# Okrio/tinyrecurrentunet

Hardware: AMD Instinct MI355X
Metric: 16 kHz frames/sec (train step) (higher is better)
Workload: dtype f32; 1 GPU; config/tiny.json TRU-Net (C_in=4 incl. PCEN), 64 x 4 s 16 kHz pairs per GPU, n_fft 512 hop 128, full fp32 train step; mfma=fp32 forward, bf16x3 backward, fp32_mfma=bf16x3-bwd, frames_per_gpu=32064, global_batch=64, parallelism=dp1

## Files before the change

tinyrecurrentunet_amd/csrc/convt_bwd.hip:

```cpp
#include <type_traits>
#include "dma_common.hpp"
#include "x3_common.hpp"

namespace {

constexpr int CT_F = 32;
constexpr int CT_C = 64;
constexpr int CT_SET = CT_C * CT_F;
constexpr int CT_GRID = TRUNET_NUM_CU;
constexpr int CT_LO = CT_C * 16;

template <int K, int S>
constexpr bool ct_dzp() { return K == 3 && S == 1; }

__device__ __forceinline__ int ct_lo_off(int r, int pc) { return r * 16 + 2 * (pc ^ ((r >> 1) & 7)); }

__device__ __forceinline__ void ct_bstore(__amdgpu_buffer_rsrc_t r, int voff, int soff, float v) {
    __builtin_amdgcn_raw_buffer_store_b32(__builtin_bit_cast(int, v), r, voff, soff, 0);
}

template <int K, int S, bool X3>
struct CtLds {
    static constexpr bool DZP = X3 && ct_dzp<K, S>();
    static constexpr int RDZ = K + 2 * S;
    static constexpr int ZS = 2 * S;
    static constexpr int RS = 4;
    static constexpr int DZ = 0;
    static constexpr int ZST = DZ + RDZ * CT_SET;
    static constexpr int SRC = ZST + ZS * CT_SET;
    static constexpr int PART = SRC + RS * CT_SET;
    static constexpr int LO = PART + 2 * 2 * 16 * 64;
    static constexpr int COEF = LO + (DZP ? RDZ * CT_LO : 0);
    static constexpr size_t BYTES = COEF * sizeof(float) + 2 * CT_C * sizeof(f32x4);
    static_assert(BYTES <= 160 * 1024, "LDS");
};

template <int K>
struct CtWtF32 { float af[K][16]; };
template <int K>
struct CtWtX3 { u32x4 A0[K][2], A1[K][2], A2[K][2]; };

template <int K, int S, bool X3>
__global__ __launch_bounds__(512, X3 ? 1 : 2) void convt_bwd_kernel(const trunet_convt_bwd_args a) {
    using L = CtLds<K, S, X3>;
    constexpr int PAD = S / 2, RDZ = L::RDZ, ZS = L::ZS, RS = L::RS;
    constexpr bool DZP = L::DZP;
    extern __shared__ __attribute__((aligned(16))) float smem[];
    float* DZ = smem + L::DZ;
    float* ZST = smem + L::ZST;
    float* SRC = smem + L::SRC;
    float* PART = smem + L::PART;
    float* LO = smem + L::LO;
    f32x4* CA = (f32x4*)(smem + L::COEF);
    f32x4* CB = CA + CT_C;

    const int tid = threadIdx.x;
    const int lane = tid & 63;
    const int wave = __builtin_amdgcn_readfirstlane(tid >> 6);
    const int h = lane >> 5, c = lane & 31;
    const int NP = a.NP, Lin = a.Lin, Lout = a.Lout;

    for (int r = tid; r < CT_C; r += 512) {
        CA[r] = f32x4{a.ca[r], a.cb[r], a.cc[r], 0.f};
        CB[r] = f32x4{a.s_scale[r], a.s_shift[r], a.s_mean[r], 0.f};
    }
    const int nfc = NP / CT_F;
    const int c_begin = (int)(((long long)blockIdx.x * nfc) / gridDim.x);
    const int c_end = (int)(((long long)(blockIdx.x + 1) * nfc) / gridDim.x);
    __syncthreads();

    if (wave < 4) {
        const int cit = wave & 1, cot = wave >> 1;
        f32x16 acc[K];
#pragma unroll
        for (int k = 0; k < K; ++k)
#pragma unroll
            for (int r = 0; r < 16; ++r) acc[k][r] = 0.f;
        float bsum[2] = {0.f, 0.f};
        const int pc = lane & 7;
        int row_[2], lc_[2];
#pragma unroll
        for (int i = 0; i < 2; ++i) {
            row_[i] = 8 * (wave + 4 * i) + (lane >> 3);
            lc_[i] = pc ^ ((row_[i] >> 1) & 7);
        }
        const float sc_a = a.s_scale[cit * 32 + c], sh_a = a.s_shift[cit * 32 + c];

        auto issue = [&](int pa, int pb, int sq, int n0) __attribute__((always_inline)) -> int {
            int n = 0;
            for (int p = max(pa, 0); p < min(pb, Lout); ++p) {
                float* dst = DZ + (p % RDZ) * CT_SET;
                float* zst = ZST + (p % ZS) * CT_SET;
#pragma unroll
                for (int i = 0; i < 2; ++i) {
                    const size_t off = ((size_t)row_[i] * Lout + p) * NP + n0 + 4 * lc_[i];
                    __builtin_amdgcn_global_load_lds(a.dy + off, (lds_ptr_t)(dst + (wave + 4 * i) * 256), 16, 0, TRUNET_DMA_AUX);
                    __builtin_amdgcn_global_load_lds(a.z + off, (lds_ptr_t)(zst + (wave + 4 * i) * 256), 16, 0, TRUNET_DMA_AUX);
                }
                n += 4;
            }
            if (sq >= 0 && sq < Lin) {
                float* sdst = SRC + (sq % RS) * CT_SET;
#pragma unroll
                for (int i = 0; i < 2; ++i) {
                    const size_t off = ((size_t)row_[i] * Lin + sq) * NP + n0 + 4 * lc_[i];
                    __builtin_amdgcn_global_load_lds(a.src + off, (lds_ptr_t)(sdst + (wave + 4 * i) * 256), 16, 0, TRUNET_DMA_AUX);
                }
                n += 2;
            }
            return n;
        };
        auto prologue = [&](int pa, int pb, int n0) __attribute__((always_inline)) {
            for (int p = max(pa, 0); p < min(pb, Lout); ++p) {
                float* dst = DZ + (p % RDZ) * CT_SET;
                const float* zst = ZST + (p % ZS) * CT_SET;
#pragma unroll
                for (int i = 0; i < 2; ++i) {
                    const int o = row_[i] * CT_F + 4 * pc;
                    f32x4 v = *(f32x4*)(dst + o);
                    const f32x4 zz = *(const f32x4*)(zst + o);
                    const f32x4 k = CA[row_[i]];
                    float s = 0.f;
#pragma unroll
                    for (int e = 0; e < 4; ++e) {
                        v[e] = fmaf(k[0], v[e], fmaf(k[1], zz[e], k[2]));
                        if (n0 + 4 * lc_[i] + e >= a.N) v[e] = 0.f;
                        s += v[e];
                    }
                    bsum[i] += s;
                    if constexpr (DZP) {
                        unsigned h0, m0, l0, h1, m1, l1;
                        ctx_split2(v[0], v[1], h0, m0, l0);
                        ctx_split2(v[2], v[3], h1, m1, l1);
                        *(u32x4*)(dst + o) = u32x4{h0, h1, m0, m1};
                        *(u32x2*)(LO + (p % RDZ) * CT_LO + row_[i] * 16 + 2 * pc) = u32x2{l0, l1};
                    } else {
                        *(f32x4*)(dst + o) = v;
                    }
                }
            }
        };
        auto new_lo = [&](int q) { return q * S - PAD + K - S; };

        constexpr int NQQ = X3 ? CT_F / 16 : CT_F / 8, QQ_PRO = X3 ? 0 : 1;

        for (int ch = c_begin; ch < c_end; ++ch) {
            const int n0 = ch * CT_F;
            {
                const int pa = -PAD, pb = new_lo(1) + S;
                for (int p = pa; p < pb; p += ZS) {
                    issue(p, min(p + ZS, pb), p == pa ? 0 : (p == pa + ZS ? 1 : -1), n0);
                    asm volatile("s_waitcnt vmcnt(0)" ::: "memory");
                    prologue(p, min(p + ZS, pb), n0);
                    asm volatile("s_waitcnt lgkmcnt(0)" ::: "memory");
                }
                if (pb - pa <= ZS) { issue(0, 0, 1, n0); asm volatile("s_waitcnt vmcnt(0)" ::: "memory"); }
            }
            int n_last = issue(new_lo(2), new_lo(2) + S, 2, n0);
            asm volatile("s_waitcnt lgkmcnt(0)" ::: "memory");
            __builtin_amdgcn_s_barrier();
            asm volatile("" ::: "memory");
            for (int q = 0; q < Lin; ++q) {
                const float* Ssrc = SRC + (q % RS) * CT_SET;
                const int ra = cit * 32 + c, rb = cot * 32 + c;
#pragma unroll
                for (int qq = 0; qq < NQQ; ++qq) {
                    if constexpr (X3) {
                        f32x4 av0 = *(const f32x4*)(Ssrc + swz_off(ra, 4 * qq + 2 * h));
                        f32x4 av1 = *(const f32x4*)(Ssrc + swz_off(ra, 4 * qq + 2 * h + 1));
#pragma unroll
                        for (int e = 0; e < 4; ++e) {
                            av0[e] = fmaxf(fmaf(av0[e], sc_a, sh_a), 0.f);
                            av1[e] = fmaxf(fmaf(av1[e], sc_a, sh_a), 0.f);
                        }
                        u32x4 a0, a1, a2;
                        ctx_split8(av0, av1, a0, a1, a2);
#pragma unroll
                        for (int k = 0; k < K; ++k) {
                            const int p = q * S - PAD + k;
                            if (p >= 0 && p < Lout) {
                                const float* Dp = DZ + (p % RDZ) * CT_SET;
                                u32x4 b0, b1, b2;
                                if constexpr (DZP) {
                                    const float* Lp = LO + (p % RDZ) * CT_LO;
                                    const u32x4 q0 = *(const u32x4*)(Dp + swz_off(rb, 4 * qq + 2 * h));
                                    const u32x4 q1 = *(const u32x4*)(Dp + swz_off(rb, 4 * qq + 2 * h + 1));
                                    const u32x2 l0 = *(const u32x2*)(Lp + ct_lo_off(rb, 4 * qq + 2 * h));
                                    const u32x2 l1 = *(const u32x2*)(Lp + ct_lo_off(rb, 4 * qq + 2 * h + 1));
                                    b0 = u32x4{q0[0], q0[1], q1[0], q1[1]};
                                    b1 = u32x4{q0[2], q0[3], q1[2], q1[3]};
                                    b2 = u32x4{l0[0], l0[1], l1[0], l1[1]};
                                } else {
                                    const f32x4 bv0 = *(const f32x4*)(Dp + swz_off(rb, 4 * qq + 2 * h));
                                    const f32x4 bv1 = *(const f32x4*)(Dp + swz_off(rb, 4 * qq + 2 * h + 1));
                                    ctx_split8(bv0, bv1, b0, b1, b2);
                                }
                                CTX_MF6(acc[k], a0, a1, a2, b0, b1, b2);
                            }
                        }
                    } else {
                        f32x4 av = *(const f32x4*)(Ssrc + swz_off(ra, 2 * qq + h));
#pragma unroll
                        for (int e = 0; e < 4; ++e) av[e] = fmaxf(fmaf(av[e], sc_a, sh_a), 0.f);
#pragma unroll
                        for (int k = 0; k < K; ++k) {
                            const int p = q * S - PAD + k;
                            if (p >= 0 && p < Lout) {
                                const f32x4 bv = *(const f32x4*)(DZ + (p % RDZ) * CT_SET + swz_off(rb, 2 * qq + h));
#pragma unroll
                                for (int j = 0; j < 4; ++j)
                                    acc[k] = __builtin_amdgcn_mfma_f32_32x32x2f32(av[j], bv[j], acc[k], 0, 0, 0);
                            }
                        }
                    }
                    if (qq == QQ_PRO && q >= 1) {
                        wait_vmcnt_exact<31>(n_last);
                        prologue(new_lo(q + 1), new_lo(q + 1) + S, n0);
                    }
                }
                asm volatile("s_waitcnt lgkmcnt(0)" ::: "memory");
                __builtin_amdgcn_s_barrier();
                asm volatile("" ::: "memory");
                n_last = (q + 3 < Lin) ? issue(new_lo(q + 3), new_lo(q + 3) + S, q + 3, n0) : 0;
            }
            asm volatile("s_waitcnt vmcnt(0)" ::: "memory");
            __builtin_amdgcn_s_barrier();
            asm volatile("" ::: "memory");
        }
        float* img = a.w_partials + (size_t)blockIdx.x * a.w_numel;
#pragma unroll
        for (int k = 0; k < K; ++k)
#pragma unroll
            for (int r = 0; r < 16; ++r) {
                const int ci = cit * 32 + (r & 3) + 8 * (r >> 2) + 4 * h;
                const int co = cot * 32 + c;
                img[((size_t)ci * CT_C + co) * K + k] = acc[k][r];
            }
        if (a.b_partials) {
#pragma unroll
            for (int i = 0; i < 2; ++i) {
                float v = bsum[i];
                v += __shfl_xor(v, 4);
                v += __shfl_xor(v, 2);
                v += __shfl_xor(v, 1);
                if ((lane & 7) == 0) a.b_partials[(size_t)blockIdx.x * a.b_stride + a.b_off + row_[i]] = v;
            }
        }
    } else {
        const int jj = wave - 4;
        const int cit = jj & 1, chf = jj >> 1;
        const int trr = 8 * (lane >> 5) + ((lane & 15) >> 2), trp = 4 * ((lane >> 4) & 1) + (lane & 3);
        std::conditional_t<X3, CtWtX3<K>, CtWtF32<K>> wt;
        if constexpr (X3) {
            const float* wp = a.W + ((size_t)(cit * 32 + c) * CT_C + chf * 32 + 8 * h) * K;
#pragma unroll
            for (int k = 0; k < K; ++k)
#pragma unroll
                for (int ks = 0; ks < 2; ++ks) {
                    f32x4 w0, w1;
#pragma unroll
                    for (int j = 0; j < 4; ++j) {
                        w0[j] = wp[(size_t)(16 * ks + j) * K + k];
                        w1[j] = wp[(size_t)(16 * ks + 4 + j) * K + k];
                    }
                    ctx_split8(w0, w1, wt.A0[k][ks], wt.A1[k][ks], wt.A2[k][ks]);
                }
        } else {
            const float* wp = a.W + ((size_t)(cit * 32 + c) * CT_C + chf * 32 + h) * K;
#pragma unroll
            for (int kk = 0; kk < 16; ++kk)
#pragma unroll
                for (int k = 0; k < K; ++k) wt.af[k][kk] = wp[(size_t)(2 * kk) * K + k];
        }
        float st1[16], st2[16];
#pragma unroll
        for (int r = 0; r < 16; ++r) { st1[r] = 0.f; st2[r] = 0.f; }
        const size_t dstride = (size_t)Lin * NP;
        const int rowb = (int)(dstride * sizeof(float));
        const int voff = (int)((4 * h * dstride + c) * sizeof(float));

        f32x16 dacc;
        auto epilogue = [&](int q, int n0) __attribute__((always_inline)) {
            const float* P = PART + ((q & 1) * 2 + cit) * 16 * 64 + lane;
            const float* Ssrc = SRC + (q % RS) * CT_SET;
            const __amdgpu_buffer_rsrc_t ro = buffer_rsrc(a.dsrc + (size_t)(32 * cit) * dstride + (size_t)q * NP);
            const bool fin = n0 + c < a.N;
            const int nb = n0 * (int)sizeof(float);
#pragma unroll
            for (int r = 0; r < 16; ++r) {
                const int ml = (r & 3) + 8 * (r >> 2);
                const int row = cit * 32 + ml + 4 * h;
                const float zs = Ssrc[row * CT_F + 4 * ((c >> 2) ^ ((row >> 1) & 7)) + (c & 3)];
                const f32x4 k = CB[row];
                float val = dacc[r] + P[r * 64];
                val = (fmaf(k[0], zs, k[1]) > 0.f) ? val : 0.f;
                ct_bstore(ro, voff, ml * rowb + nb, val);
                const float x = fin ? val : 0.f;
                st1[r] += x;
                st2[r] = fmaf(x, zs - k[2], st2[r]);
            }
        };

        for (int ch = c_begin; ch < c_end; ++ch) {
            const int n0 = wave_uniform(ch * CT_F);
            asm volatile("" ::: "memory");
            __builtin_amdgcn_s_barrier();
            asm volatile("" ::: "memory");
            for (int q = 0; q < Lin; ++q) {
#pragma unroll
                for (int r = 0; r < 16; ++r) dacc[r] = 0.f;
#pragma unroll
                for (int k = 0; k < K; ++k) {
                    const int p = q * S - PAD + k;
                    if (p < 0 || p >= Lout) continue;
                    if constexpr (DZP) {
                        const float* Dq = DZ + (p % RDZ) * CT_SET;
                        const float* Lq = LO + (p % RDZ) * CT_LO;
#pragma unroll
                        for (int ks = 0; ks < 2; ++ks) {
                            const int r0 = chf * 32 + 16 * ks + trr;
                            const u32x2 h0 = lds_tr16(Dq + swz_off(r0, trp)), h1 = lds_tr16(Dq + swz_off(r0 + 4, trp));
                            const u32x2 m0 = lds_tr16(Dq + swz_off(r0, trp) + 2), m1 = lds_tr16(Dq + swz_off(r0 + 4, trp) + 2);
                            const u32x2 l0 = lds_tr16(Lq + ct_lo_off(r0, trp)), l1 = lds_tr16(Lq + ct_lo_off(r0 + 4, trp));
                            const u32x4 b0 = {h0[0], h0[1], h1[0], h1[1]}, b1 = {m0[0], m0[1], m1[0], m1[1]},
                                        b2 = {l0[0], l0[1], l1[0], l1[1]};
                            CTX_MF6(dacc, wt.A0[k][ks], wt.A1[k][ks], wt.A2[k][ks], b0, b1, b2);
                        }
                    } else if constexpr (X3) {
                        const float* Sb = DZ + (p % RDZ) * CT_SET + (chf * 32 + 8 * h) * CT_F + (c & 3);
                        const int cpc = c >> 2;
#pragma unroll
                        for (int ks = 0; ks < 2; ++ks) {
                            f32x4 x0, x1;
#pragma unroll
                            for (int j = 0; j < 4; ++j) {
                                x0[j] = Sb[(16 * ks + j) * CT_F + 4 * (cpc ^ ((4 * h + (j >> 1)) & 7))];
                                x1[j] = Sb[(16 * ks + 4 + j) * CT_F + 4 * (cpc ^ ((4 * h + 2 + (j >> 1)) & 7))];
                            }
                            u32x4 b0, b1, b2;
                            ctx_split8(x0, x1, b0, b1, b2);
                            CTX_MF6(dacc, wt.A0[k][ks], wt.A1[k][ks], wt.A2[k][ks], b0, b1, b2);
                        }
                    } else {
                        const float* Sb = DZ + (p % RDZ) * CT_SET + (chf * 32 + h) * CT_F + (c & 3);
                        const int cpc = c >> 2;
#pragma unroll
                        for (int kk = 0; kk < 16; ++kk) {
                            const float b = Sb[kk * (2 * CT_F) + 4 * (cpc ^ (kk & 7))];
                            dacc = __builtin_amdgcn_mfma_f32_32x32x2f32(wt.af[k][kk], b, dacc, 0, 0, 0);
                        }
                    }
                }
                if (chf == 1) {
                    float* P = PART + ((q & 1) * 2 + cit) * 16 * 64 + lane;
#pragma unroll
                    for (int r = 0; r < 16; ++r) P[r * 64] = dacc[r];
                }
                asm volatile("s_waitcnt lgkmcnt(0)" ::: "memory");
                __builtin_amdgcn_s_barrier();
                asm volatile("" ::: "memory");
                if (chf == 0) epilogue(q, n0);
            }
            asm volatile("s_waitcnt lgkmcnt(0)" ::: "memory");
            __builtin_amdgcn_s_barrier();
            asm volatile("" ::: "memory");
        }
        if (chf == 0 && a.partials) {
#pragma unroll
            for (int r = 0; r < 16; ++r) {
                const float s1 = half_wave_sum(st1[r]);
                const float s2 = half_wave_sum(st2[r]);
                const int row = cit * 32 + (r & 3) + 8 * (r >> 2) + 4 * h;
                if (c == 0) {
                    float* pp = a.partials + ((size_t)blockIdx.x * CT_C + row) * 2;
                    pp[0] = s1;
                    pp[1] = s2;
                }
            }
        }
    }
}

template <int K, int S, bool X3>
int ct_launch(const trunet_convt_bwd_args* h, hipStream_t st) {
    constexpr size_t lds = CtLds<K, S, X3>::BYTES;
    auto kern = convt_bwd_kernel<K, S, X3>;
    if (hipFuncSetAttribute((const void*)kern, hipFuncAttributeMaxDynamicSharedMemorySize, (int)lds) != hipSuccess)
        return TRUNET_ELAUNCH;
    hipLaunchKernelGGL(kern, dim3(CT_GRID), dim3(512), lds, st, *h);
    return trunet_launch_status();
}
template <int K, int S>
int ct_launch(const trunet_convt_bwd_args* h, hipStream_t st, bool x3) {
    return x3 ? ct_launch<K, S, true>(h, st) : ct_launch<K, S, false>(h, st);
}

}

extern "C" int trunet_convt_bwd_nparts(void) { return CT_GRID; }

extern "C" int trunet_convt_bwd(const trunet_convt_bwd_args* h, void* stream) {
    if (!h || !h->dy || !h->z || !h->ca || !h->cb || !h->cc || !h->src || !h->s_scale || !h->s_shift || !h->s_mean ||
        !h->W || !h->dsrc || !h->partials || !h->w_partials)
        return TRUNET_EINVAL;
    if (h->NP <= 0 || (h->NP % TRUNET_TILE_FRAMES) != 0 || h->N <= 0 || h->N > h->NP || h->Lin <= 0 || h->w_numel <= 0)
        return TRUNET_EINVAL;
    if (h->Ci != CT_C || h->Co != CT_C) return TRUNET_ENOTSUP;
    if (h->pad != h->S / 2 || h->Lout != (h->Lin - 1) * h->S - 2 * h->pad + h->K) return TRUNET_EINVAL;
    if ((size_t)h->Lin * h->NP * sizeof(float) * 36 >= ((size_t)1 << 31)) return TRUNET_ENOTSUP;
    hipStream_t st = (hipStream_t)stream;
    const bool x3 = (trunet_gemm_x3_enable(-1) & (TRUNET_X3_BWD | 8)) != 0;
    if (h->K == 3 && h->S == 1) return ct_launch<3, 1>(h, st, x3);
    if (h->K == 3 && h->S == 2) return ct_launch<3, 2>(h, st, x3);
    if (h->K == 5 && h->S == 2) return ct_launch<5, 2>(h, st, x3);
    return TRUNET_ENOTSUP;
}
```

Measured before the change: 760,900 frames/s.

## Extend pre-split dz layout to all bf16x3 convT bwd shapes, shorten stride-2 lookahead

Turns on the pre-split (hi/mid/lo) dz staging in LDS for every bf16x3 transposed-conv backward variant, not only K=3,S=1. The dW and dX loops no longer re-split dz fragments for each MFMA. For stride-2 X3 kernels the load lookahead drops from two steps to one, which shrinks the dz and source ring buffers to fit the extra LO buffer in LDS. The prologue is moved to the last qq iteration so the loads have more time to land. The shorter lookahead may expose more global-load latency.

```diff
diff --git a/tinyrecurrentunet_amd/csrc/convt_bwd.hip b/tinyrecurrentunet_amd/csrc/convt_bwd.hip
--- a/tinyrecurrentunet_amd/csrc/convt_bwd.hip
+++ b/tinyrecurrentunet_amd/csrc/convt_bwd.hip
@@ -10,8 +10,8 @@
 constexpr int CT_GRID = TRUNET_NUM_CU;
 constexpr int CT_LO = CT_C * 16;
 
-template <int K, int S>
-constexpr bool ct_dzp() { return K == 3 && S == 1; }
+template <int K, int S, bool X3>
+constexpr int ct_lookahead() { return X3 && S == 2 ? 1 : 2; }
 
 __device__ __forceinline__ int ct_lo_off(int r, int pc) { return r * 16 + 2 * (pc ^ ((r >> 1) & 7)); }
 
@@ -21,10 +21,12 @@
 
 template <int K, int S, bool X3>
 struct CtLds {
-    static constexpr bool DZP = X3 && ct_dzp<K, S>();
-    static constexpr int RDZ = K + 2 * S;
-    static constexpr int ZS = 2 * S;
-    static constexpr int RS = 4;
+    static constexpr bool DZP = X3;
+    static constexpr int LA = ct_lookahead<K, S, X3>();
+    static_assert(LA == 1 || LA == 2, "the counted wait of the step loop leaves at most one issue in flight");
+    static constexpr int RDZ = K + LA * S;
+    static constexpr int ZS = LA * S;
+    static constexpr int RS = LA + 2;
     static constexpr int DZ = 0;
     static constexpr int ZST = DZ + RDZ * CT_SET;
     static constexpr int SRC = ZST + ZS * CT_SET;
@@ -43,7 +45,7 @@
 template <int K, int S, bool X3>
 __global__ __launch_bounds__(512, X3 ? 1 : 2) void convt_bwd_kernel(const trunet_convt_bwd_args a) {
     using L = CtLds<K, S, X3>;
-    constexpr int PAD = S / 2, RDZ = L::RDZ, ZS = L::ZS, RS = L::RS;
+    constexpr int PAD = S / 2, RDZ = L::RDZ, ZS = L::ZS, RS = L::RS, LA = L::LA;
     constexpr bool DZP = L::DZP;
     extern __shared__ __attribute__((aligned(16))) float smem[];
     float* DZ = smem + L::DZ;
@@ -64,6 +66,10 @@
         CA[r] = f32x4{a.ca[r], a.cb[r], a.cc[r], 0.f};
         CB[r] = f32x4{a.s_scale[r], a.s_shift[r], a.s_mean[r], 0.f};
     }
+    auto dz_slot = [](int p) __attribute__((always_inline)) {
+        if constexpr (X3 && S == 2) return wave_uniform(p % RDZ);
+        else return p % RDZ;
+    };
     const int nfc = NP / CT_F;
     const int c_begin = (int)(((long long)blockIdx.x * nfc) / gridDim.x);
     const int c_end = (int)(((long long)(blockIdx.x + 1) * nfc) / gridDim.x);
@@ -142,21 +148,21 @@
         };
         auto new_lo = [&](int q) { return q * S - PAD + K - S; };
 
-        constexpr int NQQ = X3 ? CT_F / 16 : CT_F / 8, QQ_PRO = X3 ? 0 : 1;
+        constexpr int NQQ = X3 ? CT_F / 16 : CT_F / 8, QQ_PRO = X3 ? (LA == 1 ? NQQ - 1 : 0) : 1;
 
         for (int ch = c_begin; ch < c_end; ++ch) {
             const int n0 = ch * CT_F;
             {
-                const int pa = -PAD, pb = new_lo(1) + S;
+                const int pa = -PAD, pb = new_lo(LA - 1) + S;
                 for (int p = pa; p < pb; p += ZS) {
-                    issue(p, min(p + ZS, pb), p == pa ? 0 : (p == pa + ZS ? 1 : -1), n0);
+                    issue(p, min(p + ZS, pb), p == pa ? 0 : (LA == 2 && p == pa + ZS ? 1 : -1), n0);
                     asm volatile("s_waitcnt vmcnt(0)" ::: "memory");
                     prologue(p, min(p + ZS, pb), n0);
                     asm volatile("s_waitcnt lgkmcnt(0)" ::: "memory");
                 }
-                if (pb - pa <= ZS) { issue(0, 0, 1, n0); asm volatile("s_waitcnt vmcnt(0)" ::: "memory"); }
-            }
-            int n_last = issue(new_lo(2), new_lo(2) + S, 2, n0);
+                if (LA == 2 && pb - pa <= ZS) { issue(0, 0, 1, n0); asm volatile("s_waitcnt vmcnt(0)" ::: "memory"); }
+            }
+            int n_last = issue(new_lo(LA), new_lo(LA) + S, LA, n0);
             asm volatile("s_waitcnt lgkmcnt(0)" ::: "memory");
             __builtin_amdgcn_s_barrier();
             asm volatile("" ::: "memory");
@@ -179,22 +185,15 @@
                         for (int k = 0; k < K; ++k) {
                             const int p = q * S - PAD + k;
                             if (p >= 0 && p < Lout) {
-                                const float* Dp = DZ + (p % RDZ) * CT_SET;
-                                u32x4 b0, b1, b2;
-                                if constexpr (DZP) {
-                                    const float* Lp = LO + (p % RDZ) * CT_LO;
-                                    const u32x4 q0 = *(const u32x4*)(Dp + swz_off(rb, 4 * qq + 2 * h));
-                                    const u32x4 q1 = *(const u32x4*)(Dp + swz_off(rb, 4 * qq + 2 * h + 1));
-                                    const u32x2 l0 = *(const u32x2*)(Lp + ct_lo_off(rb, 4 * qq + 2 * h));
-                                    const u32x2 l1 = *(const u32x2*)(Lp + ct_lo_off(rb, 4 * qq + 2 * h + 1));
-                                    b0 = u32x4{q0[0], q0[1], q1[0], q1[1]};
-                                    b1 = u32x4{q0[2], q0[3], q1[2], q1[3]};
-                                    b2 = u32x4{l0[0], l0[1], l1[0], l1[1]};
-                                } else {
-                                    const f32x4 bv0 = *(const f32x4*)(Dp + swz_off(rb, 4 * qq + 2 * h));
-                                    const f32x4 bv1 = *(const f32x4*)(Dp + swz_off(rb, 4 * qq + 2 * h + 1));
-                                    ctx_split8(bv0, bv1, b0, b1, b2);
-                                }
+                                const int sl = dz_slot(p);
+                                const float* Dp = DZ + sl * CT_SET;
+                                const float* Lp = LO + sl * CT_LO;
+                                const u32x4 q0 = *(const u32x4*)(Dp + swz_off(rb, 4 * qq + 2 * h));
+                                const u32x4 q1 = *(const u32x4*)(Dp + swz_off(rb, 4 * qq + 2 * h + 1));
+                                const u32x2 l0 = *(const u32x2*)(Lp + ct_lo_off(rb, 4 * qq + 2 * h));
+                                const u32x2 l1 = *(const u32x2*)(Lp + ct_lo_off(rb, 4 * qq + 2 * h + 1));
+                                const u32x4 b0 = {q0[0], q0[1], q1[0], q1[1]}, b1 = {q0[2], q0[3], q1[2], q1[3]},
+                                            b2 = {l0[0], l0[1], l1[0], l1[1]};
                                 CTX_MF6(acc[k], a0, a1, a2, b0, b1, b2);
                             }
                         }
@@ -213,15 +212,15 @@
                             }
                         }
                     }
-                    if (qq == QQ_PRO && q >= 1) {
-                        wait_vmcnt_exact<31>(n_last);
+                    if (qq == QQ_PRO && q >= LA - 1) {
+                        wait_vmcnt_exact<31>(LA == 2 ? n_last : 0);
                         prologue(new_lo(q + 1), new_lo(q + 1) + S, n0);
                     }
                 }
                 asm volatile("s_waitcnt lgkmcnt(0)" ::: "memory");
                 __builtin_amdgcn_s_barrier();
                 asm volatile("" ::: "memory");
-                n_last = (q + 3 < Lin) ? issue(new_lo(q + 3), new_lo(q + 3) + S, q + 3, n0) : 0;
+                n_last = (q + 1 + LA < Lin) ? issue(new_lo(q + 1 + LA), new_lo(q + 1 + LA) + S, q + 1 + LA, n0) : 0;
             }
             asm volatile("s_waitcnt vmcnt(0)" ::: "memory");
             __builtin_amdgcn_s_barrier();
@@ -314,8 +313,9 @@
                     const int p = q * S - PAD + k;
                     if (p < 0 || p >= Lout) continue;
                     if constexpr (DZP) {
-                        const float* Dq = DZ + (p % RDZ) * CT_SET;
-                        const float* Lq = LO + (p % RDZ) * CT_LO;
+                        const int sl = dz_slot(p);
+                        const float* Dq = DZ + sl * CT_SET;
+                        const float* Lq = LO + sl * CT_LO;
 #pragma unroll
                         for (int ks = 0; ks < 2; ++ks) {
                             const int r0 = chf * 32 + 16 * ks + trr;
@@ -324,21 +324,6 @@
                             const u32x2 l0 = lds_tr16(Lq + ct_lo_off(r0, trp)), l1 = lds_tr16(Lq + ct_lo_off(r0 + 4, trp));
                             const u32x4 b0 = {h0[0], h0[1], h1[0], h1[1]}, b1 = {m0[0], m0[1], m1[0], m1[1]},
                                         b2 = {l0[0], l0[1], l1[0], l1[1]};
-                            CTX_MF6(dacc, wt.A0[k][ks], wt.A1[k][ks], wt.A2[k][ks], b0, b1, b2);
-                        }
-                    } else if constexpr (X3) {
-                        const float* Sb = DZ + (p % RDZ) * CT_SET + (chf * 32 + 8 * h) * CT_F + (c & 3);
-                        const int cpc = c >> 2;
-#pragma unroll
-                        for (int ks = 0; ks < 2; ++ks) {
-                            f32x4 x0, x1;
-#pragma unroll
-                            for (int j = 0; j < 4; ++j) {
-                                x0[j] = Sb[(16 * ks + j) * CT_F + 4 * (cpc ^ ((4 * h + (j >> 1)) & 7))];
-                                x1[j] = Sb[(16 * ks + 4 + j) * CT_F + 4 * (cpc ^ ((4 * h + 2 + (j >> 1)) & 7))];
-                            }
-                            u32x4 b0, b1, b2;
-                            ctx_split8(x0, x1, b0, b1, b2);
                             CTX_MF6(dacc, wt.A0[k][ks], wt.A1[k][ks], wt.A2[k][ks], b0, b1, b2);
                         }
                     } else {
```

Result: faster. 769,100 frames/s (median of 6 runs) (+1.1%).
